# ctpeterson/qex

Hardware: AMD Instinct MI355X
Metric: staggered Dslash GFLOP/s + CG iters/s, 32^4 SU(3) fp64, 1/2/4/8 MI355X (higher is better)
Workload: dtype f64

## Files before the change

profiles/summarize.py:

```python
import csv
import glob
import json
import os
import re
import shutil
import sys
from collections import defaultdict

outdir, tag = sys.argv[1], sys.argv[2]
VOL = 32 ** 4
for d in sorted(glob.glob(os.path.join(outdir, "trace_*"))):
    name = os.path.basename(d)[len("trace_"):]
    for f in glob.glob(os.path.join(d, "**", "*kernel_stats.csv"), recursive=True):
        shutil.copy(f, os.path.join(outdir, "%s_%s_kernel_stats.csv" % (tag, name)))


def split_name(full):
    s = full.strip()
    s = re.sub(r"^void\s+", "", s)
    m = re.match(r"([A-Za-z_][A-Za-z0-9_:]*)", s)
    fn = m.group(1) if m else s
    rest = s[len(fn):]
    targs = ""
    if rest.startswith("<"):
# ... 65 lines not shown
    return (tot / n, n, lo, hi) if n else (None, 0, None, None)


GiB = 1024.0 ** 3
rd, _ = mean("k_read16", None, "FETCH_SIZE")
cp_w, _ = mean("k_copy16", None, "WRITE_SIZE")
if rd and cp_w:
    fcorr = GiB / (rd * 1024.0)
    wcorr = GiB / (cp_w * 1024.0)
    note = ("HBM bytes per launch = FETCH_SIZE*1024*fetch_correction + WRITE_SIZE*1024*write_correction, dispatch-weighted means over "
            "the dispatches of profiles/pmc_workload.py; corrections from the 1 GiB k_read16 / k_copy16 kernels of the same passes; "
            "kernels matched by exact function name and template arguments")
    tj = {"source": "profiles/collect.sh " + tag, "fetch_correction": fcorr, "write_correction": wcorr, "note": note}
    for fn, targs, key in (("k_dslash", "<8, false, false, false, 0>", "dslash8_sweep1_18real"), ("k_dslash", "<8, false, true, true, 0>", "dslash8_sweep2_18real"),
                           ("k_dslash", "<8, false, false, false, 1>", "dslash8_sweep1_recon12"), ("k_dslash", "<8, false, true, true, 1>", "dslash8_sweep2_recon12"),
                           ("k_dslash", "<16, false, false, false, 0>", "dslash16_sweep1_18real"), ("k_dslash", "<16, false, true, true, 0>", "dslash16_sweep2_18real")):
        fe, _ = mean(fn, targs, "FETCH_SIZE")
        wr, _ = mean(fn, targs, "WRITE_SIZE")
        if fe is not None and wr is not None:
            tj[key + "_bytes"] = fe * 1024.0 * fcorr + wr * 1024.0 * wcorr
    if "dslash8_sweep1_18real_bytes" in tj and "dslash8_sweep2_18real_bytes" in tj:
        tj["hbm_bytes_per_launch_32x4"] = 0.5 * (tj["dslash8_sweep1_18real_bytes"] + tj["dslash8_sweep2_18real_bytes"])
    if "dslash8_sweep1_recon12_bytes" in tj and "dslash8_sweep2_recon12_bytes" in tj:
        tj["hbm_bytes_per_launch_32x4_recon12"] = 0.5 * (tj["dslash8_sweep1_recon12_bytes"] + tj["dslash8_sweep2_recon12_bytes"])
    json.dump(tj, open(os.path.join(outdir, "%s_dslash_traffic.json" % tag), "w"), indent=1)

    Vh = VOL // 2
    M = 144
    priced = [
        ("k_dslash", "<8, false, false, false, 0>", (8 * M + 48 + 48) * Vh, "8 links + vector in + vector out per output site (SURVEY 8d: 1248 B)"),
        ("k_dslash", "<8, false, true, true, 0>", (8 * M + 48 + 48 + 48) * Vh, "the same + the 4 m^2 x term (1296 B)"),
        ("k_dslash", "<16, false, false, false, 0>", (16 * M + 48 + 48) * Vh, "16 links + vector in + out (2400 B)"),
        ("k_dslash", "<16, false, true, true, 0>", (16 * M + 48 + 48 + 48) * Vh, "the same + the 4 m^2 x term"),
        ("k_cg_xpay", None, 144 * Vh, "p = r + beta p: 2 reads + 1 write of 48 B"),
        ("k_cg_update", None, 288 * Vh, "x, r updates: 4 reads + 2 writes of 48 B"),
        ("k_cgm_update", None, (48 + 96 + 9 * 192) * Vh, "r in, ps[0] in/out, 9 x (xs, ps in/out), 10 shifts"),
        ("k_force_lds", None, (4 * M * 3 + 4 * M * 2.0 / 3.0) * VOL, "U in, U' out, momentum out, momentum in for stages 2-3 (2112 B/site average)"),
        ("k_force_lds2", None, (4 * M * 3 + 4 * M * 2.0 / 3.0) * VOL, "U in, U' out, momentum out, momentum in for stages 2-3 (2112 B/site average); both parities of a tile position per workgroup"),
        ("k_plaq", None, 4 * M * VOL, "4 links per site read once (576 B)"),
        ("k_flow_obs_clover", None, 4 * M * VOL, "4 links per site read once (576 B)"),
        ("k_flow_obs_clover2", None, 4 * M * VOL, "4 links per site read once (576 B): plaquettes + clover E, Q in one pass, both parities of a tile position per workgroup"),
        ("k_flow_obs_all", None, 4 * M * VOL, "4 links per site read once (576 B): plaquette + clover E, Q in one pass"),
        ("k_gen_staple", None, 4 * M * VOL, "two input matrices read once, accumulator read + written: 576 B/site unique"),
        ("k_staple_deriv_pair", None, 10 * M * VOL, "a (mu,nu)/(nu,mu) pair: 6 matrices read, 2 read and written back = 1440 B/site (rounds 2-3 quoted the 8 reads alone, 1152 B, against read + write traffic)"),
        ("k_projUderiv_batch", None, None, "864 B per link of the batch (sizes differ per level: see dispatches)"),
    ]
    kt = {"source": "profiles/collect.sh " + tag + " (profiles/pmc_workload.py, 32^4)", "fetch_correction": fcorr, "write_correction": wcorr,
          "note": note + "; avg_us from the --kernel-trace --stats pass of the same workload; achieved_alg_gbs = alg_bytes / avg_us", "kernels": {}}
    for fn, targs, alg, what in priced:
        fe, nfe = mean(fn, targs, "FETCH_SIZE")
        wr, _ = mean(fn, targs, "WRITE_SIZE")
        if fe is None or wr is None:
            continue
        hbm_r, hbm_w = fe * 1024.0 * fcorr, wr * 1024.0 * wcorr
        us, ncalls, lo, hi = avg_us(fn, targs)
        e = {"dispatches_pmc": nfe, "hbm_read_bytes": round(hbm_r), "hbm_write_bytes": round(hbm_w), "hbm_bytes": round(hbm_r + hbm_w), "what_alg_counts": what}
        if alg is not None:
            e["alg_bytes"] = int(alg)
            e["ratio_hbm_over_alg"] = round((hbm_r + hbm_w) / alg, 3)
        if us:
            e.update({"avg_us": round(us, 2), "min_us": round(lo, 2), "max_us": round(hi, 2), "calls_trace": ncalls})
            if alg is not None:
                e["achieved_alg_gbs"] = round(alg / us / 1e3, 1)
                e["frac_of_8TBs"] = round(alg / us / 1e3 / 8000.0, 4)
            e["achieved_hbm_gbs"] = round((hbm_r + hbm_w) / us / 1e3, 1)
        for extra in ("TCC_HIT_sum", "TCC_MISS_sum", "TCP_TCC_READ_REQ_sum"):
            v, _ = mean(fn, targs, extra)
            if v is not None:
# ... 5 lines not shown
```

qex_amd/csrc/api.cpp:

```cpp
#include "qexhip_internal.h"
#include <string>
#include "../../include/qexhip.h"
#include <algorithm>
#include <cmath>
#include <cstdarg>
#include <cstdlib>
#include <cstring>
#include <vector>

static thread_local char g_err[1024] = "";

void qexhip_set_error(const char *fmt, ...) {
  va_list ap;
  va_start(ap, fmt);
  vsnprintf(g_err, sizeof(g_err), fmt, ap);
  va_end(ap);
}
extern "C" const char *qexhip_last_error(void) { return g_err; }

static bool timer_class_on(const qexhip_ctx *c, const char *name) {
  if (!c->timers_on) return false;
  if (c->timers_on == 2) return strncmp(name, "dslash", 6) == 0;
  if (c->timers_on == 3) return strncmp(name, "dslash", 6) == 0 || strcmp(name, "exchange") == 0 || strcmp(name, "allreduce") == 0;
  return true;
// ... 57 lines not shown
  return 0;
}

static int init_body(qexhip_ctx *c, int device, const int latLocal[4], const int rankGeom[4], const int rankCoord[4]) {
  int ndev = 0;
  HIPCHK(hipGetDeviceCount(&ndev));
  if (ndev <= 0) { qexhip_set_error("no HIP device visible: libqexhip has no CPU fallback"); return QEXHIP_ERR_HIP; }
  if (device < 0 || device >= ndev) { qexhip_set_error("device %d out of range (%d visible)", device, ndev); return QEXHIP_ERR_ARG; }
  c->device = device;
  for (int i = 0; i < 4; i++) {
    c->rankGeom[i] = rankGeom ? rankGeom[i] : 1;
    c->rankCoord[i] = rankCoord ? rankCoord[i] : 0;
  }
  for (int i = 0; i < 3; i++)
    if (c->rankGeom[i] != 1) { qexhip_set_error("only rankGeom = {1,1,1,N} (split along t) is supported"); return QEXHIP_ERR_ARG; }
  const int halo = c->rankGeom[3] > 1;
  if (geom_init(c->g, latLocal, 1, halo)) return QEXHIP_ERR_ARG;
  HIPCHK(hipSetDevice(device));
  HIPCHK(hipStreamCreateWithFlags(&c->stream, hipStreamNonBlocking));
  {
    int lo = 0, hi = 0;
    if (hipDeviceGetStreamPriorityRange(&lo, &hi) == hipSuccess && hi != lo) HIPCHK(hipStreamCreateWithPriority(&c->cstream, hipStreamNonBlocking, hi));
    else HIPCHK(hipStreamCreateWithFlags(&c->cstream, hipStreamNonBlocking));
  }
  HIPCHK(hipEventCreateWithFlags(&c->ev_ready, hipEventDisableTiming));
  c->part2_off = std::max(6144, (c->g.Vh + 255) / 256 + 8);
  c->npartials = c->part2_off + 2048 + 64;
  HIPCHK(hipMalloc((void **)&c->partials, sizeof(double) * c->npartials));
  HIPCHK(hipMalloc((void **)&c->dscal, sizeof(double) * 64));
  HIPCHK(hipMemset(c->dscal, 0, sizeof(double) * 64));
  HIPCHK(hipMalloc((void **)&c->cg, sizeof(CgScal)));
  HIPCHK(hipMemset(c->cg, 0, sizeof(CgScal)));
  HIPCHK(hipHostMalloc(&c->pinned, 4096, hipHostMallocDefault));
  CHK(devjoin_init(c));
  if (getenv("QEXHIP_TEST_FAIL_INIT")) {
    qexhip_set_error("QEXHIP_TEST_FAIL_INIT: injected failure");
    return QEXHIP_ERR_HIP;
  }
  if (const char *e = getenv("QEXHIP_OVERLAP")) c->opt_overlap = atoi(e);
  if (const char *e = getenv("QEXHIP_HOP_SPLIT")) { const int v = atoi(e); c->opt_hop_split = v < 0 ? -1 : (v ? 2 : 0); }
  if (const char *e = getenv("QEXHIP_RECON")) c->opt_recon = atoi(e);
  if (const char *e = getenv("QEXHIP_FLOW_EXP")) c->opt_flow_exp = atoi(e);
  {
    int a = 0, b = 0;
    (void)hipDeviceGetAttribute(&a, hipDeviceAttributeMaxSharedMemoryPerBlock, device);
    (void)hipDeviceGetAttribute(&b, hipDeviceAttributeSharedMemPerBlockOptin, device);
    (void)hipGetLastError();
    const int lds = a > b ? a : b;
    if (lds < 147456 + 1024) {
      qexhip_set_error("device %d offers %d bytes of LDS per workgroup; libqexhip is built for gfx950 (160 KiB)", device, lds);
      return QEXHIP_ERR_STATE;
    }
  }
  c->nranks = 1;
  c->rank = 0;
  return 0;
}

extern "C" int qexhip_init(qexhip_handle *h, int device, const int latLocal[4], const int rankGeom[4],
                           const int rankCoord[4]) {
  if (!h || !latLocal) return QEXHIP_ERR_ARG;
  qexhip_ctx *c = new qexhip_ctx();
  const int e = init_body(c, device, latLocal, rankGeom, rankCoord);
  if (e) {
    (void)qexhip_finalize(c);
    return e;
// ... 19 lines not shown
  for (auto &kv : c->timers) for (auto e : kv.second.ev) (void)hipEventDestroy(e);
  nhyp_state_free(c);
  hisq_state_free(c);
  batch_state_free(c);
  batch_f32_state_free(c);
  batch_half_state_free(c);
  msf_state_free(c);
  gfix_state_free(c);
  stout_state_free(c);
  eig_state_free(c);
  eig_bases_free(c);
  for (auto &kv : c->cfields) (void)hipFree(kv.second.d);
  c->cfields.clear();
  gauge_free(c);
  comm_destroy(c);
  if (c->W) (void)hipFree(c->W);
  f32_state_free(c);
  half_state_free(c);
  if (c->outer_F) (void)hipFree(c->outer_F);
  if (c->obs_table) (void)hipFree(c->obs_table);
  if (c->tile_order) (void)hipFree(c->tile_order);
  for (int *&t : c->tile_order_pl) if (t) { (void)hipFree(t); t = nullptr; }
  if (c->cgm_scal) (void)hipFree(c->cgm_scal);
  if (c->meson_buf) (void)hipFree(c->meson_buf);
  if (c->Wc) (void)hipFree(c->Wc);
  if (c->Ws) (void)hipFree(c->Ws);
  if (c->Wm) (void)hipFree(c->Wm);
  if (c->stage) (void)hipFree(c->stage);
  if (c->partials) (void)hipFree(c->partials);
  if (c->dscal) (void)hipFree(c->dscal);
  if (c->cg) (void)hipFree(c->cg);
  if (c->hist) (void)hipFree(c->hist);
  if (c->pinned) (void)hipHostFree(c->pinned);
  if (c->fz_buf) (void)hipFree(c->fz_buf);
  devjoin_destroy(c);
  if (c->ev_ready) (void)hipEventDestroy(c->ev_ready);
  if (c->stream) (void)hipStreamDestroy(c->stream);
  if (c->cstream) (void)hipStreamDestroy(c->cstream);
  (void)hipGetLastError();
  delete c;
  return 0;
}

extern "C" int qexhip_sync(qexhip_handle c) {
  if (!c) return QEXHIP_ERR_ARG;
  CHK(devjoin_flush(c));
  HIPCHK(hipStreamSynchronize(c->cstream));
  HIPCHK(hipStreamSynchronize(c->stream));
  return devjoin_check(c);
}

extern "C" int qexhip_device_info(qexhip_handle c, char *buf, int buflen) {
  if (!c || !buf) return QEXHIP_ERR_ARG;
  hipDeviceProp_t p;
  HIPCHK(hipGetDeviceProperties(&p, c->device));
  int n = snprintf(buf, buflen, "%s (%s) CUs=%d mem=%.0fGiB local=%dx%dx%dx%d ranks=%d halo=%d tile_pairs=%d", p.name, p.gcnArchName,
                   p.multiProcessorCount, p.totalGlobalMem / 1073741824.0, c->g.X[0], c->g.X[1], c->g.X[2], c->g.X[3],
                   c->rankGeom[3], c->g.halo, c->tile_order ? c->tile_pairs_ok : -1);
  if (c->g.halo && c->W && n > 0 && n < buflen) {
    double t[8];
    if (qexhip_stag_sweep_tuning(c, t) == 0)
      snprintf(buf + n, buflen - n, "; sweep: overlap=%d form=%s exchange=%.1fus%s boundary_at=%.2f spin=%.0fus tuned[first|sites|fused]=%.0f|%.0f|%.0f us",
               (int)t[7], t[5] == 2 ? "fused" : "by-sites", t[0], c->xchg_us[c->ndir == 16] > 0 ? "(measured)" : "(estimate)", t[1], t[6], t[2], t[3], t[4]);
  }
  return 0;
}
// ... 1438 lines not shown
```

qex_amd/csrc/blas.hip:

```cpp
#include "qexhip_internal.h"
#include "reduce.h"
#include "cg_device.h"
#include <cstring>
#include "peer_device.h"

static inline int grid_for(size_t n2) {
  size_t nb = (n2 + 255) / 256;
  if (nb > 2048) nb = 2048;
  if (nb < 1) nb = 1;
  return (int)nb;
}
static inline size_t body2(const qexhip_ctx *c) { return (size_t)c->g.ntile * 192; }

#define FOR_PAR(par, p) for (int p = ((par) == 2 ? 0 : (par)); p <= ((par) == 2 ? 1 : (par)); p++)

__global__ void __launch_bounds__(256) k_zero(double2 *y, size_t n) {
  for (size_t i = blockIdx.x * 256 + threadIdx.x; i < n; i += (size_t)gridDim.x * 256) y[i] = make_double2(0, 0);
}
__global__ void __launch_bounds__(256) k_copy(double2 *y, const double2 *x, size_t n) {
  for (size_t i = blockIdx.x * 256 + threadIdx.x; i < n; i += (size_t)gridDim.x * 256) y[i] = x[i];
}
__global__ void __launch_bounds__(256) k_axpy(double a, const double2 *x, double2 *y, size_t n) {
  for (size_t i = blockIdx.x * 256 + threadIdx.x; i < n; i += (size_t)gridDim.x * 256) {
    double2 xv = x[i], yv = y[i];
// ... 137 lines not shown
  if (threadIdx.x == 0) out[blockIdx.x] = r;
}
int blas_cdot(qexhip_ctx *c, const DevField &x, const DevField &y, int parity, double *dev_out) {
  size_t n = body2(c);
  const int nb = grid_for(n);
  int tot = 0;
  double *pre = c->partials, *pim = c->partials + 2 * nb;
  if (4 * nb > c->part2_off + 2048) { qexhip_set_error("internal: partial buffer too small for cdot"); return -3; }
  {
    ScopedTimer tm(c, "blas", c->stream);
    FOR_PAR(parity, p) {
      k_cdot<<<nb, 256, 0, c->stream>>>(x.par(p), y.par(p), n, pre + tot, pim + tot);
      tot += nb;
    }
    k_reduce_final2<<<2, 256, 0, c->stream>>>(pre, pim, tot, dev_out);
    HIPCHK(hipGetLastError());
  }
  if (multi_rank(c)) CHK(comm_allreduce(c, dev_out, 2));
  return 0;
}

int blas_norm2(qexhip_ctx *c, const DevField &x, int parity, double *dev_out) {
  return blas_redot(c, x, x, parity, dev_out);
}

int read_scalars(qexhip_ctx *c, const double *dev, int n, double *host) {
  HIPCHK(hipMemcpyAsync(c->pinned, dev, sizeof(double) * n, hipMemcpyDeviceToHost, c->stream));
  HIPCHK(hipStreamSynchronize(c->stream));
  CHK(peer_check(c));
  for (int i = 0; i < n; i++) host[i] = ((double *)c->pinned)[i];
  return 0;
}

__global__ void __launch_bounds__(256) k_cg_xpay(double2 *p, const double2 *r, size_t n, CgScal *s, int k, int rolled,
                                                const double *r2parts, int nparts, double *hist, int histcap) {
  const int cur = k & 1, prv = cur ^ 1;
  double r2k;
  if (rolled) {
    if (s->dones[cur]) return;
    r2k = s->r2s[cur];
  } else {
    if (s->dones[prv]) {
      if (blockIdx.x == 0 && threadIdx.x == 0) cg_carry(s, k);
      return;
    }
    r2k = cg_sum_parts(r2parts, nparts);
    if (blockIdx.x == 0 && threadIdx.x == 0) cg_roll(s, k, r2k, hist, histcap);
    if (!(k < s->maxits && r2k > s->r2stop)) return;
  }
  const bool first = (k == 0);
  const double beta = r2k / s->r2s[prv];
  for (size_t i = blockIdx.x * 256 + threadIdx.x; i < n; i += (size_t)gridDim.x * 256) {
    double2 rv = r[i];
    if (first) p[i] = rv;
    else {
      double2 pv = p[i];
      p[i] = make_double2(fma(beta, pv.x, rv.x), fma(beta, pv.y, rv.y));
    }
  }
}
__global__ void __launch_bounds__(256) k_cg_update(double2 *x, double2 *r, const double2 *p, const double2 *Ap,
                                                  size_t n, const CgScal *s, int k, double *partials,
                                                  const double *dotp, int ndot) {
  if (s->dones[k & 1]) return;
  const double pAp = (ndot > 0) ? cg_sum_parts(dotp, ndot) : s->pAp;
  const double alpha = s->r2s[k & 1] / pAp;
  double acc = 0;
  for (size_t i = blockIdx.x * 256 + threadIdx.x; i < n; i += (size_t)gridDim.x * 256) {
    double2 pv = p[i], xv = x[i], rv = r[i], av = Ap[i];
    xv.x += alpha * pv.x; xv.y += alpha * pv.y;
    rv.x -= alpha * av.x; rv.y -= alpha * av.y;
    x[i] = xv; r[i] = rv;
    acc = fma(rv.x, rv.x, fma(rv.y, rv.y, acc));
  }
  double t = block_sum_256(acc);
  if (threadIdx.x == 0) partials[blockIdx.x] = t;
}
__global__ void k_cg_init(CgScal *s, const double *dscal, double r2req, int maxits, double *hist, int histcap) {
  s->b2 = dscal[0];
  s->r2 = dscal[1];
  s->rzo = 1.0;
  s->pAp = 0.0;
  s->r2stop = r2req * s->b2;
  s->itn = 0;
  s->maxits = maxits;
  s->done = !(0 < maxits && s->r2 > s->r2stop);
  s->r2s[0] = s->r2; s->itns[0] = 0; s->dones[0] = s->done;
  s->r2s[1] = 1.0; s->itns[1] = 0; s->dones[1] = s->done;
  if (histcap > 0) hist[0] = (s->b2 != 0.0) ? s->r2 / s->b2 : 0.0;
}
__global__ void __launch_bounds__(256) k_cg_close(CgScal *s, int k, const double *r2parts, int nparts, double *hist, int histcap) {
  if (s->dones[(k & 1) ^ 1]) {
    if (threadIdx.x == 0) cg_carry(s, k);
    return;
  }
  const double r2k = cg_sum_parts(r2parts, nparts);
  if (threadIdx.x == 0) cg_roll(s, k, r2k, hist, histcap);
}

int cg_xpay(qexhip_ctx *c, DevField &p, const DevField &r, int parity, int k, int rolled) {
  size_t n = body2(c);
  ScopedTimer tm(c, "blas", c->stream);
  k_cg_xpay<<<grid_for(n), 256, 0, c->stream>>>(p.par(parity), r.par(parity), n, c->cg, k, rolled,
                                               c->partials + c->part2_off, rolled ? grid_for(n) : c->cg_r2parts, c->hist, c->histcap);
  HIPCHK(hipGetLastError());
  return 0;
}
int cg_update(qexhip_ctx *c, DevField &x, DevField &r, const DevField &p, const DevField &Ap, int parity, int k, int ndot) {
  size_t n = body2(c);
  int nb = grid_for(n);
  double *r2p = c->partials + c->part2_off;
  if (ndot > 0) CHK(comm_allreduce_parts(c, c->partials, ndot, &ndot));
  CHK(devjoin_flush(c));
  {
    ScopedTimer tm(c, "blas", c->stream);
    k_cg_update<<<nb, 256, 0, c->stream>>>(x.par(parity), r.par(parity), p.par(parity), Ap.par(parity), n, c->cg, k, r2p,
                                           c->partials, ndot);
    HIPCHK(hipGetLastError());
  }
  CHK(comm_allreduce_parts(c, r2p, nb, &c->cg_r2parts));
  return 0;
}
int cg_close(qexhip_ctx *c, int k) {
  k_cg_close<<<1, 256, 0, c->stream>>>(c->cg, k, c->partials + c->part2_off, c->cg_r2parts, c->hist, c->histcap);
  HIPCHK(hipGetLastError());
  return comm_agree_post(c);
}
__global__ void k_cg_resume(CgScal *s, int k, double r2req, int maxits) {
  const int cur = k & 1;
  s->r2stop = r2req * s->b2;
  s->maxits = maxits;
  s->r2s[cur] = s->r2; s->r2s[cur ^ 1] = s->rzo; s->itns[cur] = k;
  s->dones[cur] = !(k < maxits && s->r2s[cur] > s->r2stop);
  s->done = s->dones[cur];
  s->agree[0] = s->r2s[cur]; s->agree[1] = -s->r2s[cur]; s->agree[2] = (double)k; s->agree[3] = -(double)k;
}
int cg_resume(qexhip_ctx *c, int k, double r2req, int maxits) {
  k_cg_resume<<<1, 1, 0, c->stream>>>(c->cg, k, r2req, maxits);
  HIPCHK(hipGetLastError());
  return 0;
}
int cg_init(qexhip_ctx *c, double r2req, int maxits) {
  c->cg_resume.valid = 0;
  k_cg_init<<<1, 1, 0, c->stream>>>(c->cg, c->dscal, r2req, maxits, c->hist, c->histcap);
  HIPCHK(hipGetLastError());
  return 0;
}
```

qex_amd/csrc/qexhip_internal.h:

```cpp
#pragma once
#include <hip/hip_runtime.h>
#include <cstdint>
#include <cstdio>
#include <string>
#include <vector>
#include <map>

#define QEXHIP_TILE 64

struct Geom {
  int X[4];
  int Xh;
  int V, Vh;
  int F;
  int ntile;
  int depth;
  int gtile;
  int etile;
  int halo;
};

__host__ __device__ inline size_t vec_off(int pos, int colour) {
  return (size_t)(pos >> 6) * 192 + (size_t)colour * 64 + (size_t)(pos & 63);
}
// ... 7 lines not shown
  double2 *d = nullptr;
  size_t half = 0;
  double2 *par(int p) const { return d + (size_t)p * half; }
};

struct DevFieldF {
  float2 *d = nullptr;
  size_t half = 0;
  float2 *par(int p) const { return d + (size_t)p * half; }
};

struct DevCField {
  double2 *d = nullptr;
  size_t half = 0;
  double2 *par(int p) const { return d + (size_t)p * half; }
};

struct SlpScal {
  double b2, r2stop;
  double r2t;
  double sigma, sigma_p;
  double r2s, r2s_old, maxr2s;
  int k, maxits, nupd;
  int done, upd, noupd;
  int conv, first;
};

struct CgScal {
  double b2, r2, rzo, pAp, r2stop, tmp;
  int itn, maxits, done, pad;
  double r2s[2];
  int itns[2], dones[2];
  double agree[4];
};

struct TimerSlot {
  std::vector<hipEvent_t> ev;
  size_t used = 0;
  long count = 0;
  double total_ms = 0;
};

struct DevJoin {
  unsigned long long *ready = nullptr;
  unsigned long long *err = nullptr;
  long long ticks = 0;
  double timeout_s = 30.0;
  unsigned long long seq[2]{0, 0};
  int deferred = 0;
};

struct GaugeNat {
  double2 *U = nullptr, *F = nullptr, *P = nullptr;
  double2 *U2 = nullptr;
  double2 *D2 = nullptr;
  size_t n2 = 0;
  int ghost_valid = 0;
  double *pp = nullptr; int npp = 0;
  double2 *M = nullptr;
  double2 *Usave = nullptr;
  int save_ghost_valid = 0;
};
struct PeerComm;

struct EigBasis {
  double2 *v = nullptr;
// ... 2 lines not shown
  unsigned long gen = 0;
  std::vector<double> evals;
  int nevals = 0;
};

enum { WK_SLOTS = 16 };

struct qexhip_ctx {
  int device = 0;
  Geom g{};
  int rankGeom[4]{1, 1, 1, 1}, rankCoord[4]{0, 0, 0, 0};
  hipStream_t stream = nullptr, cstream = nullptr;
  hipEvent_t ev_ready = nullptr;
  void *comm = nullptr;
  void *comm2 = nullptr;
  PeerComm *peer = nullptr;
  DevJoin dj;
  int opt_transport = -1;
  int nranks = 1, rank = 0;
  int force_halo = 0;
  double2 *W = nullptr;
  int ndir = 0;
  std::map<int, DevField> fields;
  int next_field = 1;
  double *stage = nullptr; size_t stage_bytes = 0;
  double *partials = nullptr; int npartials = 0;
  int part2_off = 0;
  double *dscal = nullptr;
  CgScal *cg = nullptr;
  struct { int valid = 0; const double2 *x = nullptr; int par_even = 0; double m2 = 0; int k = 0; } cg_resume;
  int cg_r2parts = 0;
  double *hist = nullptr; int histcap = 0;
  void *pinned = nullptr;
  int wk[WK_SLOTS]{0};
  int timers_on = 0;
  std::map<std::string, TimerSlot> timers;
  double2 *Wc = nullptr; unsigned long long *Ws = nullptr; size_t Wc_rows = 0; int recon = 0; double recon_dev = 0;
  unsigned long long *Wm = nullptr; size_t Wm_rows = 0; int lres = 0; long long lres_esc = 0;
  int opt_lossless = 3;
  int opt_batch_multi = 0;
  int opt_multi_reduce = 0;
  int opt_force_pair = 1;
  int opt_obs_clover = 1;
  int opt_hop_split = -1;
  int opt_fused_spin_us = -1;
  int ranks_share_device = 0;
  int hybrid_sums = 0;
  unsigned int *fz_buf = nullptr; int fz_cap = 0;
  const double2 *bnd_out_on_cstream = nullptr;
  double xchg_us[2]{0, 0};
  int form_auto[2]{-1, -1};
  int opt_chain_overlap = 1;
  int opt_hisq_md_fused = 3;
  int opt_smear_ca = 1;
  int opt_flow_exp = 1;
  int opt_recon = 2;
  int opt_overlap = -1;
  int emu_link_gbs = 0;
  int emu_exchange_us = 0, emu_allreduce_us = 0;
  int overlap_auto[2]{-1, -1};
  double overlap_tune_us[2][3]{};
  GaugeNat *gn = nullptr;
  void *nhyp = nullptr;
  void *hisq = nullptr;
  double2 *outer_F = nullptr; size_t outer_Fn = 0;
  int tile_pairs_ok = 0;
// ... 181 lines not shown
int half_pack_host(const double *v, size_t nsites, int16_t *q, float *norm);
int half_unpack_host(const int16_t *q, const float *norm, size_t nsites, double *v);
int half_links(qexhip_ctx *c, int *fmt, double *s_fat, double *s_long, double *dev);
int half_op_xx_probe(qexhip_ctx *c, DevField &fr, const DevField &fx, double m2, int par_even);
int slph_begin(qexhip_ctx *c, SlpScal *s);
int slph_iterate(qexhip_ctx *c, SlpScal *s, DevFieldF &xs, const DevField &r, double m2, int par_even);
int slph_stall(qexhip_ctx *c, SlpScal *s, int limit);
int slph_stalled(qexhip_ctx *c, int *stalled);
void half_state_free(qexhip_ctx *c);

#define CGM_MAXM 32
void msf_state_free(qexhip_ctx *c);
int msf_r2_buffer(qexhip_ctx *c, double **dev);
int msf_start(qexhip_ctx *c, SlpScal *s, DevFieldF &rs, const DevField &b, std::vector<DevField *> &xs, const double *shifts, int nmass,
              int parity, DevFieldF **ps0);
int msf_iterate(qexhip_ctx *c, SlpScal *s, DevFieldF &rs, const DevFieldF &Ap, const DevField &r, int parity, int ndot);
int msf_flush(qexhip_ctx *c, SlpScal *s, int nmass);

int blas_zero(qexhip_ctx *c, DevField &f, int parity);
int blas_copy(qexhip_ctx *c, DevField &dst, const DevField &src, int parity);
int blas_axpy(qexhip_ctx *c, double a, const DevField &x, DevField &y, int parity);
int blas_xpay(qexhip_ctx *c, const DevField &x, double a, DevField &y, int parity);
int blas_scale(qexhip_ctx *c, double a, DevField &y, int parity);
int blas_axpby(qexhip_ctx *c, double a, const DevField &x, double b, const DevField &y, DevField &z, int parity);
int blas_norm2(qexhip_ctx *c, const DevField &x, int parity, double *dev_out);
int blas_redot(qexhip_ctx *c, const DevField &x, const DevField &y, int parity, double *dev_out);
int blas_cdot(qexhip_ctx *c, const DevField &x, const DevField &y, int parity, double *dev_out);
int tile_order_table(qexhip_ctx *c, const int **tab, int *chunk);
int tile_order_plane(qexhip_ctx *c, int mu, int nu, const int **tab, int *chunk);
int reduce_partials(qexhip_ctx *c, int n, double *dev_out);
int read_scalars(qexhip_ctx *c, const double *dev, int n, double *host);
int blas_grid(const qexhip_ctx *c, int parity_count);
int blas_delay(hipStream_t st, int us);
int cg_xpay(qexhip_ctx *c, DevField &p, const DevField &r, int parity, int k, int rolled);
int cg_update(qexhip_ctx *c, DevField &x, DevField &r, const DevField &p, const DevField &Ap, int parity, int k, int ndot);
int cg_close(qexhip_ctx *c, int k);
int cg_init(qexhip_ctx *c, double r2req, int maxits);
int cg_resume(qexhip_ctx *c, int k, double r2req, int maxits);

int get_work(qexhip_ctx *c, int slot, DevField **f);
int op_xx(qexhip_ctx *c, DevField &r, DevField &x, double m2, int par_even, int dot, const int *done, int *ndot = nullptr);
int op_D(qexhip_ctx *c, DevField &r, DevField &x, double m, double sc, double a = 0.0);
int norm2_eo(qexhip_ctx *c, DevField &f, double *e, double *o);
int resid_eo(qexhip_ctx *c, DevField &r, DevField &b, DevField &x, double m, double *e, double *o);
int solve_xx_dev(qexhip_ctx *c, DevField &x, DevField &b, double mass, double r2req, int maxits,
                 int par_even, int *iters, double *r2_over_b2, double *hist, int histcap);
int solve_xx_continue_dev(qexhip_ctx *c, DevField &x, double r2req, int maxits, int *iters, double *r2_over_b2, double *hist, int histcap);
int solve_full_dev(qexhip_ctx *c, DevField &x, DevField &b, double mass, double r2req, int maxits,
                   int *iters, double *r2_final, int use_prev = 0, int sloppy = 0, int *nupdates = nullptr);
int solve_xx_sloppy_dev(qexhip_ctx *c, DevField &x, DevField &b, double mass, double r2req, int maxits, int par_even,
                        int *iters, double *r2_over_b2, int *nupdates);
int solve_xx_half_dev(qexhip_ctx *c, DevField &x, DevField &b, double mass, double r2req, int maxits, int par_even,
                      int *iters, double *r2_over_b2, int *nupdates);
int half_finish_f32(qexhip_ctx *c, DevField &x, DevField &b, const DevField &r, DevField &Ax, double mass, double r2stop, int maxits,
                    int par_even, double *r2t, int *its32, int *nupd32);
int solve_xx_sloppy_any(qexhip_ctx *c, int sloppy, DevField &x, DevField &b, double mass, double r2req, int maxits, int par_even,
                        int *iters, double *r2_over_b2, int *nupdates);
int solve_xx_multi_dev(qexhip_ctx *c, std::vector<DevField *> &xs, DevField &b, const double *shifts,
                       int nmass, double r2req, int maxits, int par_even, int *iters, double *hist, int histcap);
int solve_multi_dev(qexhip_ctx *c, std::vector<DevField *> &xs, DevField &b, const double *masses,
                    int nmass, double r2req, int maxits, int *iters, double *r2_final, int sloppy = 0, int *nupdates = nullptr);
int multi_sloppy_check(qexhip_ctx *c, int sloppy, const double *vals, int nmass);
int solve_xx_multi_sloppy_dev(qexhip_ctx *c, std::vector<DevField *> &xs, DevField &b, const double *shifts, int nmass, double r2req,
                              int maxits, int par_even, int *iters, double *r2_over_b2, int *nupdates, int *refine_iters);
enum { POOL_PS = 0, POOL_YS = 32, POOL_XS = 64, POOL_REF = 96 };
int pool_field(qexhip_ctx *c, int idx, DevField **f);
int rational_map(const char *who, double mass, int nterm, const double *alpha, const double *beta, double *shifts, int *order);
int rational_xx_dev(qexhip_ctx *c, DevField &out, DevField &b, double mass, double f0, int nterm, const double *alpha, const double *beta,
                    double r2req, int maxits, int par_even, int *iters, double *hist, int histcap);
// ... 127 lines not shown
```

qex_amd/csrc/solver.cpp:

```cpp
#include "qexhip_internal.h"
#include "full_solve.h"
#include "../../include/qexhip.h"
#include <cmath>
#include <cstring>
#include <algorithm>
#include <vector>


int get_work(qexhip_ctx *c, int slot, DevField **f) {
  if (slot == WK_R || slot == WK_P || slot == WK_AP) c->cg_resume.valid = 0;
  if (c->wk[slot] == 0) {
    DevField nf;
    CHK(field_alloc(c, nf));
    int id = -(slot + 1);
    c->fields[id] = nf;
    c->wk[slot] = id;
  }
  *f = &c->fields[c->wk[slot]];
  return 0;
}

int op_xx(qexhip_ctx *c, DevField &r, DevField &x, double m2, int par_even, int dot, const int *done, int *ndot) {
  DevField *t;
  CHK(get_work(c, WK_T, &t));
  const int px = par_even ? 0 : 1, py = 1 - px;
  DslashOpts o1, o2;
  o1.done = done;
  o2.cb = 4.0 * m2;
  o2.xs = &x;
  o2.neg = 1;
  o2.dot = (dot && ndot) ? 2 : dot;
  o2.nparts_out = ndot;
  o2.dot_out = &c->cg->pAp;
  o2.done = done;
// ... 16 lines not shown
}

int op_D(qexhip_ctx *c, DevField &r, DevField &x, double m, double sc, double a) {
  CHK(op_stagD(c, r, x, 0, m, sc, a));
  CHK(op_stagD(c, r, x, 1, m, sc, a));
  return 0;
}

static int op_eo_reconstruct(qexhip_ctx *c, DevField &r, DevField &b, double m) {
  CHK(op_stagD(c, r, r, 1, 0.0, -1.0 / m, 0.0));
  CHK(blas_axpy(c, 1.0 / m, b, r, 1));
  return 0;
}
int op_eo_reconstruct_pub(qexhip_ctx *c, DevField &r, DevField &b, double m) { return op_eo_reconstruct(c, r, b, m); }
int op_stagD_pub(qexhip_ctx *c, DevField &r, DevField &x, int parity, double m, double sc, double a) { return op_stagD(c, r, x, parity, m, sc, a); }
int op_eo_reduce_pub(qexhip_ctx *c, DevField &r, DevField &b, double m) { return op_stagD(c, r, b, 0, m, -1.0, 0.0); }

static int ensure_hist(qexhip_ctx *c, int cap) {
  if (cap < 1) cap = 1;
  if (c->histcap >= cap) return 0;
  if (c->hist) HIPCHK(hipFree(c->hist));
  c->hist = nullptr; c->histcap = 0;
  HIPCHK(hipMalloc((void **)&c->hist, sizeof(double) * cap));
  c->histcap = cap;
  return 0;
}

static int read_cg(qexhip_ctx *c, CgScal *host) {
  HIPCHK(hipMemcpyAsync(c->pinned, c->cg, sizeof(CgScal), hipMemcpyDeviceToHost, c->stream));
  HIPCHK(hipStreamSynchronize(c->stream));
  memcpy(host, c->pinned, sizeof(CgScal));
  return 0;
}

static int cg_iterate(qexhip_ctx *c, DevField &x, DevField *r, DevField *p, DevField *Ap, double m2, int par_even, int k,
                      CgScal &st, int *iters, double *r2_over_b2, double *hist, int histcap) {
  const int par = par_even ? 0 : 1;
  const int chunk = 32;
  int rolled = 1;
  bool done = st.dones[k & 1];
  double r2 = st.r2s[k & 1];
  st.itn = st.itns[k & 1];
  while (!done) {
    int n = std::min(chunk, st.maxits - k);
    if (n <= 0) break;
    for (int i = 0; i < n; i++, k++) {
      CHK(cg_xpay(c, *p, *r, par, k, rolled));
      rolled = 0;
      int ndot = 0;
      CHK(op_xx(c, *Ap, *p, m2, par_even, 1, &c->cg->dones[k & 1], &ndot));
      CHK(cg_update(c, x, *r, *p, *Ap, par, k, ndot));
    }
    CHK(cg_close(c, k));
    rolled = 1;
    CHK(read_cg(c, &st));
    CHK(comm_agree_check(c, st));
    done = st.dones[k & 1];
    r2 = st.r2s[k & 1];
    st.itn = st.itns[k & 1];
  }
  st.r2 = r2;
  if (iters) *iters = st.itn;
  if (r2_over_b2) *r2_over_b2 = (st.b2 != 0.0) ? st.r2 / st.b2 : 0.0;
  if (hist && histcap > 0) {
    int n = std::min(std::min(histcap, c->histcap), st.itn + 1);
    HIPCHK(hipMemcpyAsync(hist, c->hist, sizeof(double) * n, hipMemcpyDeviceToHost, c->stream));
    HIPCHK(hipStreamSynchronize(c->stream));
  }
  c->cg_resume.valid = 1; c->cg_resume.x = x.d; c->cg_resume.par_even = par_even; c->cg_resume.m2 = m2; c->cg_resume.k = st.itn;
  return 0;
}

int solve_xx_dev(qexhip_ctx *c, DevField &x, DevField &b, double mass, double r2req, int maxits,
                 int par_even, int *iters, double *r2_over_b2, double *hist, int histcap) {
  const int par = par_even ? 0 : 1;
  DevField *r, *p, *Ap;
  CHK(get_work(c, WK_R, &r));
  CHK(get_work(c, WK_P, &p));
  CHK(get_work(c, WK_AP, &Ap));
  CHK(ensure_hist(c, std::max(histcap, 1)));
  const double m2 = mass * mass;
  CHK(blas_zero(c, x, 2));
  CHK(blas_norm2(c, b, par, &c->dscal[0]));
  CHK(blas_copy(c, *r, b, par));
  CHK(blas_norm2(c, *r, par, &c->dscal[1]));
  CHK(cg_init(c, r2req, maxits));
  CgScal st;
  CHK(read_cg(c, &st));
  return cg_iterate(c, x, r, p, Ap, m2, par_even, 0, st, iters, r2_over_b2, hist, histcap);
}

int solve_xx_continue_dev(qexhip_ctx *c, DevField &x, double r2req, int maxits, int *iters, double *r2_over_b2, double *hist, int histcap) {
// ... 527 lines not shown
```

Before: 3012.

## Defer CG x update into next xpay and post chunk-end reads ahead

The CG x += alpha p update moves out of k_cg_update into the next iteration's k_cg_xpay, or into k_cg_close at a chunk end. alpha is stored in CgScal for that purpose. This shrinks the update kernel's traffic and fuses the x stream with the p stream. The chunk-end host read of the CG scalars now goes through an event with double-buffered pinned slots, and two iterations of the next chunk are enqueued before the host waits, so the GPU does not sit idle during the convergence check. The cost is a close kernel that now sweeps the whole field, and up to two extra speculative iterations, which are gated on device by the done flags.

```diff
diff --git a/profiles/summarize.py b/profiles/summarize.py
--- a/profiles/summarize.py
+++ b/profiles/summarize.py
@@ -121,8 +121,8 @@
         ("k_dslash", "<8, false, true, true, 0>", (8 * M + 48 + 48 + 48) * Vh, "the same + the 4 m^2 x term (1296 B)"),
         ("k_dslash", "<16, false, false, false, 0>", (16 * M + 48 + 48) * Vh, "16 links + vector in + out (2400 B)"),
         ("k_dslash", "<16, false, true, true, 0>", (16 * M + 48 + 48 + 48) * Vh, "the same + the 4 m^2 x term"),
-        ("k_cg_xpay", None, 144 * Vh, "p = r + beta p: 2 reads + 1 write of 48 B"),
-        ("k_cg_update", None, 288 * Vh, "x, r updates: 4 reads + 2 writes of 48 B"),
+        ("k_cg_xpay", None, 240 * Vh, "x += alpha p of the iteration before, p = r + beta p: 3 reads + 2 writes of 48 B"),
+        ("k_cg_update", None, 144 * Vh, "r update: 2 reads + 1 write of 48 B"),
         ("k_cgm_update", None, (48 + 96 + 9 * 192) * Vh, "r in, ps[0] in/out, 9 x (xs, ps in/out), 10 shifts"),
         ("k_force_lds", None, (4 * M * 3 + 4 * M * 2.0 / 3.0) * VOL, "U in, U' out, momentum out, momentum in for stages 2-3 (2112 B/site average)"),
         ("k_force_lds2", None, (4 * M * 3 + 4 * M * 2.0 / 3.0) * VOL, "U in, U' out, momentum out, momentum in for stages 2-3 (2112 B/site average); both parities of a tile position per workgroup"),
diff --git a/qex_amd/csrc/api.cpp b/qex_amd/csrc/api.cpp
--- a/qex_amd/csrc/api.cpp
+++ b/qex_amd/csrc/api.cpp
@@ -113,6 +113,7 @@
   HIPCHK(hipMalloc((void **)&c->cg, sizeof(CgScal)));
   HIPCHK(hipMemset(c->cg, 0, sizeof(CgScal)));
   HIPCHK(hipHostMalloc(&c->pinned, 4096, hipHostMallocDefault));
+  for (hipEvent_t &e : c->cg_ev) HIPCHK(hipEventCreateWithFlags(&e, hipEventDisableTiming));
   CHK(devjoin_init(c));
   if (getenv("QEXHIP_TEST_FAIL_INIT")) {
     qexhip_set_error("QEXHIP_TEST_FAIL_INIT: injected failure");
@@ -198,6 +199,7 @@
   if (c->cg) (void)hipFree(c->cg);
   if (c->hist) (void)hipFree(c->hist);
   if (c->pinned) (void)hipHostFree(c->pinned);
+  for (hipEvent_t e : c->cg_ev) if (e) (void)hipEventDestroy(e);
   if (c->fz_buf) (void)hipFree(c->fz_buf);
   devjoin_destroy(c);
   if (c->ev_ready) (void)hipEventDestroy(c->ev_ready);
diff --git a/qex_amd/csrc/blas.hip b/qex_amd/csrc/blas.hip
--- a/qex_amd/csrc/blas.hip
+++ b/qex_amd/csrc/blas.hip
@@ -193,46 +193,80 @@
   return 0;
 }
 
-__global__ void __launch_bounds__(256) k_cg_xpay(double2 *p, const double2 *r, size_t n, CgScal *s, int k, int rolled,
+
+__device__ __forceinline__ double2 cg_xup(double alpha, double2 pv, double2 xv) {
+  return make_double2(fma(alpha, pv.x, xv.x), fma(alpha, pv.y, xv.y));
+}
+
+__global__ void __launch_bounds__(256) k_cg_xpay(double2 *x, double2 *p, const double2 *r, size_t n, CgScal *s, int k, int rolled,
                                                 const double *r2parts, int nparts, double *hist, int histcap) {
   const int cur = k & 1, prv = cur ^ 1;
-  double r2k;
+  const size_t stride = (size_t)gridDim.x * 256;
+  size_t i = blockIdx.x * 256 + threadIdx.x;
+  const bool first = (k == 0), pend = !rolled;
+  double2 rv = make_double2(0, 0), pv = rv, xv = rv;
+  if (i < n) {
+    rv = r[i];
+    if (!first) pv = p[i];
+    if (pend) xv = x[i];
+  }
+  const int done_prv = s->dones[prv], maxits = s->maxits;
+  const double r2prv = s->r2s[prv], r2stop = s->r2stop, alpha = s->alphas[prv];
+  const int done_cur = rolled ? s->dones[cur] : 0;
+  double r2k = rolled ? s->r2s[cur] : 0.0;
+  bool go = true;
   if (rolled) {
-    if (s->dones[cur]) return;
-    r2k = s->r2s[cur];
+    if (done_cur) return;
   } else {
-    if (s->dones[prv]) {
+    if (done_prv) {
       if (blockIdx.x == 0 && threadIdx.x == 0) cg_carry(s, k);
       return;
     }
     r2k = cg_sum_parts(r2parts, nparts);
     if (blockIdx.x == 0 && threadIdx.x == 0) cg_roll(s, k, r2k, hist, histcap);
-    if (!(k < s->maxits && r2k > s->r2stop)) return;
-  }
-  const bool first = (k == 0);
-  const double beta = r2k / s->r2s[prv];
-  for (size_t i = blockIdx.x * 256 + threadIdx.x; i < n; i += (size_t)gridDim.x * 256) {
-    double2 rv = r[i];
+    go = (k < maxits && r2k > r2stop);
+  }
+  if (!go) {
+    while (i < n) {
+      x[i] = cg_xup(alpha, pv, xv);
+      i += stride;
+      if (i < n) { pv = p[i]; xv = x[i]; }
+    }
+    return;
+  }
+  const double beta = r2k / r2prv;
+  while (i < n) {
+    if (pend) x[i] = cg_xup(alpha, pv, xv);
     if (first) p[i] = rv;
-    else {
-      double2 pv = p[i];
-      p[i] = make_double2(fma(beta, pv.x, rv.x), fma(beta, pv.y, rv.y));
-    }
-  }
-}
-__global__ void __launch_bounds__(256) k_cg_update(double2 *x, double2 *r, const double2 *p, const double2 *Ap,
-                                                  size_t n, const CgScal *s, int k, double *partials,
+    else p[i] = make_double2(fma(beta, pv.x, rv.x), fma(beta, pv.y, rv.y));
+    i += stride;
+    if (i < n) {
+      rv = r[i];
+      if (!first) pv = p[i];
+      if (pend) xv = x[i];
+    }
+  }
+}
+__global__ void __launch_bounds__(256) k_cg_update(double2 *r, const double2 *Ap, size_t n, CgScal *s, int k, double *partials,
                                                   const double *dotp, int ndot) {
-  if (s->dones[k & 1]) return;
-  const double pAp = (ndot > 0) ? cg_sum_parts(dotp, ndot) : s->pAp;
-  const double alpha = s->r2s[k & 1] / pAp;
+  const int cur = k & 1;
+  const size_t stride = (size_t)gridDim.x * 256;
+  size_t i = blockIdx.x * 256 + threadIdx.x;
+  double2 rv = make_double2(0, 0), av = rv;
+  if (i < n) { rv = r[i]; av = Ap[i]; }
+  const int done = s->dones[cur];
+  const double r2 = s->r2s[cur], pAp0 = s->pAp;
+  if (done) return;
+  const double pAp = (ndot > 0) ? cg_sum_parts(dotp, ndot) : pAp0;
+  const double alpha = r2 / pAp;
+  if (blockIdx.x == 0 && threadIdx.x == 0) s->alphas[cur] = alpha;
   double acc = 0;
-  for (size_t i = blockIdx.x * 256 + threadIdx.x; i < n; i += (size_t)gridDim.x * 256) {
-    double2 pv = p[i], xv = x[i], rv = r[i], av = Ap[i];
-    xv.x += alpha * pv.x; xv.y += alpha * pv.y;
+  while (i < n) {
     rv.x -= alpha * av.x; rv.y -= alpha * av.y;
-    x[i] = xv; r[i] = rv;
+    r[i] = rv;
     acc = fma(rv.x, rv.x, fma(rv.y, rv.y, acc));
+    i += stride;
+    if (i < n) { rv = r[i]; av = Ap[i]; }
   }
   double t = block_sum_256(acc);
   if (threadIdx.x == 0) partials[blockIdx.x] = t;
@@ -250,24 +284,39 @@
   s->r2s[1] = 1.0; s->itns[1] = 0; s->dones[1] = s->done;
   if (histcap > 0) hist[0] = (s->b2 != 0.0) ? s->r2 / s->b2 : 0.0;
 }
-__global__ void __launch_bounds__(256) k_cg_close(CgScal *s, int k, const double *r2parts, int nparts, double *hist, int histcap) {
-  if (s->dones[(k & 1) ^ 1]) {
-    if (threadIdx.x == 0) cg_carry(s, k);
+__global__ void __launch_bounds__(256) k_cg_close(double2 *x, const double2 *p, size_t n, CgScal *s, int k, const double *r2parts,
+                                                 int nparts, double *hist, int histcap) {
+  const int prv = (k & 1) ^ 1;
+  const size_t stride = (size_t)gridDim.x * 256;
+  size_t i = blockIdx.x * 256 + threadIdx.x;
+  double2 pv = make_double2(0, 0), xv = pv;
+  if (i < n) { pv = p[i]; xv = x[i]; }
+  const int done_prv = s->dones[prv];
+  const double alpha = s->alphas[prv];
+  if (done_prv) {
+    if (blockIdx.x == 0 && threadIdx.x == 0) cg_carry(s, k);
     return;
   }
-  const double r2k = cg_sum_parts(r2parts, nparts);
-  if (threadIdx.x == 0) cg_roll(s, k, r2k, hist, histcap);
-}
-
-int cg_xpay(qexhip_ctx *c, DevField &p, const DevField &r, int parity, int k, int rolled) {
+  if (blockIdx.x == 0) {
+    const double r2k = cg_sum_parts(r2parts, nparts);
+    if (threadIdx.x == 0) cg_roll(s, k, r2k, hist, histcap);
+  }
+  while (i < n) {
+    x[i] = cg_xup(alpha, pv, xv);
+    i += stride;
+    if (i < n) { pv = p[i]; xv = x[i]; }
+  }
+}
+
+int cg_xpay(qexhip_ctx *c, DevField &x, DevField &p, const DevField &r, int parity, int k, int rolled) {
   size_t n = body2(c);
   ScopedTimer tm(c, "blas", c->stream);
-  k_cg_xpay<<<grid_for(n), 256, 0, c->stream>>>(p.par(parity), r.par(parity), n, c->cg, k, rolled,
+  k_cg_xpay<<<grid_for(n), 256, 0, c->stream>>>(x.par(parity), p.par(parity), r.par(parity), n, c->cg, k, rolled,
                                                c->partials + c->part2_off, rolled ? grid_for(n) : c->cg_r2parts, c->hist, c->histcap);
   HIPCHK(hipGetLastError());
   return 0;
 }
-int cg_update(qexhip_ctx *c, DevField &x, DevField &r, const DevField &p, const DevField &Ap, int parity, int k, int ndot) {
+int cg_update(qexhip_ctx *c, DevField &r, const DevField &Ap, int parity, int k, int ndot) {
   size_t n = body2(c);
   int nb = grid_for(n);
   double *r2p = c->partials + c->part2_off;
@@ -275,15 +324,16 @@
   CHK(devjoin_flush(c));
   {
     ScopedTimer tm(c, "blas", c->stream);
-    k_cg_update<<<nb, 256, 0, c->stream>>>(x.par(parity), r.par(parity), p.par(parity), Ap.par(parity), n, c->cg, k, r2p,
-                                           c->partials, ndot);
+    k_cg_update<<<nb, 256, 0, c->stream>>>(r.par(parity), Ap.par(parity), n, c->cg, k, r2p, c->partials, ndot);
     HIPCHK(hipGetLastError());
   }
   CHK(comm_allreduce_parts(c, r2p, nb, &c->cg_r2parts));
   return 0;
 }
-int cg_close(qexhip_ctx *c, int k) {
-  k_cg_close<<<1, 256, 0, c->stream>>>(c->cg, k, c->partials + c->part2_off, c->cg_r2parts, c->hist, c->histcap);
+int cg_close(qexhip_ctx *c, DevField &x, const DevField &p, int parity, int k) {
+  size_t n = body2(c);
+  k_cg_close<<<grid_for(n), 256, 0, c->stream>>>(x.par(parity), p.par(parity), n, c->cg, k, c->partials + c->part2_off, c->cg_r2parts,
+                                                c->hist, c->histcap);
   HIPCHK(hipGetLastError());
   return comm_agree_post(c);
 }
diff --git a/qex_amd/csrc/cg_posting.h b/qex_amd/csrc/cg_posting.h
--- /dev/null
+++ b/qex_amd/csrc/cg_posting.h
@@ -0,0 +1,28 @@
+#pragma once
+#include <vector>
+
+enum { CG_POST_ITERS = 0, CG_POST_CLOSE = 1, CG_POST_WAIT = 2 };
+struct CgPostStep {
+  int kind, k, n;
+};
+
+inline std::vector<CgPostStep> cg_posting_plan(int k, int maxits, int chunk, int ahead) {
+  std::vector<CgPostStep> plan;
+  if (chunk < 1) chunk = 1;
+  if (ahead < 0) ahead = 0;
+  if (ahead > chunk) ahead = chunk;
+  int n = maxits - k < chunk ? maxits - k : chunk;
+  if (n <= 0) return plan;
+  plan.push_back({CG_POST_ITERS, k, n});
+  k += n;
+  for (;;) {
+    plan.push_back({CG_POST_CLOSE, k, 0});
+    n = maxits - k < chunk ? maxits - k : chunk;
+    const int a = n < ahead ? (n > 0 ? n : 0) : ahead;
+    if (a > 0) plan.push_back({CG_POST_ITERS, k, a});
+    plan.push_back({CG_POST_WAIT, k, 0});
+    if (n <= 0) return plan;
+    if (n > a) plan.push_back({CG_POST_ITERS, k + a, n - a});
+    k += n;
+  }
+}
diff --git a/qex_amd/csrc/qexhip_internal.h b/qex_amd/csrc/qexhip_internal.h
--- a/qex_amd/csrc/qexhip_internal.h
+++ b/qex_amd/csrc/qexhip_internal.h
@@ -63,6 +63,7 @@
   double r2s[2];
   int itns[2], dones[2];
   double agree[4];
+  double alphas[2];
 };
 
 struct TimerSlot {
@@ -131,6 +132,7 @@
   int cg_r2parts = 0;
   double *hist = nullptr; int histcap = 0;
   void *pinned = nullptr;
+  hipEvent_t cg_ev[2]{nullptr, nullptr};
   int wk[WK_SLOTS]{0};
   int timers_on = 0;
   std::map<std::string, TimerSlot> timers;
@@ -378,9 +380,9 @@
 int read_scalars(qexhip_ctx *c, const double *dev, int n, double *host);
 int blas_grid(const qexhip_ctx *c, int parity_count);
 int blas_delay(hipStream_t st, int us);
-int cg_xpay(qexhip_ctx *c, DevField &p, const DevField &r, int parity, int k, int rolled);
-int cg_update(qexhip_ctx *c, DevField &x, DevField &r, const DevField &p, const DevField &Ap, int parity, int k, int ndot);
-int cg_close(qexhip_ctx *c, int k);
+int cg_xpay(qexhip_ctx *c, DevField &x, DevField &p, const DevField &r, int parity, int k, int rolled);
+int cg_update(qexhip_ctx *c, DevField &r, const DevField &Ap, int parity, int k, int ndot);
+int cg_close(qexhip_ctx *c, DevField &x, const DevField &p, int parity, int k);
 int cg_init(qexhip_ctx *c, double r2req, int maxits);
 int cg_resume(qexhip_ctx *c, int k, double r2req, int maxits);
 
diff --git a/qex_amd/csrc/solver.cpp b/qex_amd/csrc/solver.cpp
--- a/qex_amd/csrc/solver.cpp
+++ b/qex_amd/csrc/solver.cpp
@@ -1,5 +1,6 @@
 #include "qexhip_internal.h"
 #include "full_solve.h"
+#include "cg_posting.h"
 #include "../../include/qexhip.h"
 #include <cmath>
 #include <cstring>
@@ -82,32 +83,52 @@
   memcpy(host, c->pinned, sizeof(CgScal));
   return 0;
 }
+static_assert(sizeof(CgScal) <= 512, "two CgScal slots in the pinned scratch");
+static int post_read_cg(qexhip_ctx *c, int slot) {
+  HIPCHK(hipMemcpyAsync((char *)c->pinned + 512 * slot, c->cg, sizeof(CgScal), hipMemcpyDeviceToHost, c->stream));
+  HIPCHK(hipEventRecord(c->cg_ev[slot], c->stream));
+  return 0;
+}
+static int wait_read_cg(qexhip_ctx *c, int slot, CgScal *host) {
+  HIPCHK(hipEventSynchronize(c->cg_ev[slot]));
+  memcpy(host, (char *)c->pinned + 512 * slot, sizeof(CgScal));
+  return 0;
+}
 
 static int cg_iterate(qexhip_ctx *c, DevField &x, DevField *r, DevField *p, DevField *Ap, double m2, int par_even, int k,
                       CgScal &st, int *iters, double *r2_over_b2, double *hist, int histcap) {
   const int par = par_even ? 0 : 1;
   const int chunk = 32;
+  const int ahead = 2;
   int rolled = 1;
   bool done = st.dones[k & 1];
   double r2 = st.r2s[k & 1];
   st.itn = st.itns[k & 1];
-  while (!done) {
-    int n = std::min(chunk, st.maxits - k);
-    if (n <= 0) break;
-    for (int i = 0; i < n; i++, k++) {
-      CHK(cg_xpay(c, *p, *r, par, k, rolled));
-      rolled = 0;
-      int ndot = 0;
-      CHK(op_xx(c, *Ap, *p, m2, par_even, 1, &c->cg->dones[k & 1], &ndot));
-      CHK(cg_update(c, x, *r, *p, *Ap, par, k, ndot));
-    }
-    CHK(cg_close(c, k));
-    rolled = 1;
-    CHK(read_cg(c, &st));
-    CHK(comm_agree_check(c, st));
-    done = st.dones[k & 1];
-    r2 = st.r2s[k & 1];
-    st.itn = st.itns[k & 1];
+  if (!done) {
+    int slot = 0;
+    for (const CgPostStep &ps : cg_posting_plan(k, st.maxits, chunk, ahead)) {
+      if (ps.kind == CG_POST_ITERS) {
+        for (k = ps.k; k < ps.k + ps.n; k++) {
+          CHK(cg_xpay(c, x, *p, *r, par, k, rolled));
+          rolled = 0;
+          int ndot = 0;
+          CHK(op_xx(c, *Ap, *p, m2, par_even, 1, &c->cg->dones[k & 1], &ndot));
+          CHK(cg_update(c, *r, *Ap, par, k, ndot));
+        }
+      } else if (ps.kind == CG_POST_CLOSE) {
+        CHK(cg_close(c, x, *p, par, ps.k));
+        rolled = 1;
+        slot ^= 1;
+        CHK(post_read_cg(c, slot));
+      } else {
+        CHK(wait_read_cg(c, slot, &st));
+        CHK(comm_agree_check(c, st));
+        done = st.dones[ps.k & 1];
+        r2 = st.r2s[ps.k & 1];
+        st.itn = st.itns[ps.k & 1];
+        if (done) break;
+      }
+    }
   }
   st.r2 = r2;
   if (iters) *iters = st.itn;
diff --git a/scratch/timeline_chunk_end.py b/scratch/timeline_chunk_end.py
--- /dev/null
+++ b/scratch/timeline_chunk_end.py
@@ -0,0 +1,44 @@
+import csv, glob, statistics, sys
+d = sys.argv[1]
+f = glob.glob(d + "/**/*kernel_trace.csv", recursive=True)[0]
+rows = list(csv.DictReader(open(f)))
+short = lambda n: n.split("(")[0].replace("void ", "")[:44]
+ev = sorted((int(r["Start_Timestamp"]), int(r["End_Timestamp"]), short(r["Kernel_Name"])) for r in rows)
+cg = ("k_cg_xpay", "k_dslash", "k_cg_update", "k_cg_close")
+closes = [i for i, e in enumerate(ev) if e[2].startswith("k_cg_close")]
+spans = []
+for i in closes:
+    nxt = [j for j in range(i + 1, min(i + 8, len(ev))) if ev[j][2].startswith("k_cg_xpay")]
+    if not ev[i - 1][2].startswith("k_cg_update") or not nxt:
+        continue
+    j = nxt[0]
+    if any(not (ev[m][2].startswith("__amd_rocclr_copyBuffer")) for m in range(i + 1, j)):
+        continue
+    busy = sum(ev[m][1] - ev[m][0] for m in range(i, j))
+    spans.append((i, j, (ev[j][0] - ev[i - 1][1] - busy) / 1e3, (ev[j][0] - ev[i - 1][1]) / 1e3))
+print("chunk ends inside a solve: %d" % len(spans))
+if spans:
+    idle = [s[2] for s in spans]
+    wall = [s[3] for s in spans]
+    print("  update end -> next xpay start: median %.1f us (min %.1f, max %.1f); of it idle (no kernel running): median %.1f us (min %.1f, max %.1f)"
+          % (statistics.median(wall), min(wall), max(wall), statistics.median(idle), min(idle), max(idle)))
+    which = int(sys.argv[2]) if len(sys.argv) > 2 else len(spans) - 1
+    i, j = spans[which][0], spans[which][1]
+    t0 = ev[i - 4][0]
+    print("  one of them (start, end, duration, gap in front; us):")
+    for m in range(i - 4, min(j + 5, len(ev))):
+        s, e, n = ev[m]
+        print("  %9.1f %9.1f  %7.1f  gap %6.1f  %s" % ((s - t0) / 1e3, (e - t0) / 1e3, (e - s) / 1e3, (s - ev[m - 1][1]) / 1e3, n))
+gaps, durs = {}, {}
+for a, b in zip(ev, ev[1:]):
+    if a[2].startswith(cg) and b[2].startswith(cg) and not a[2].startswith("k_cg_close") and not b[2].startswith("k_cg_close"):
+        gaps.setdefault(a[2][:28] + " -> " + b[2][:28], []).append((b[0] - a[1]) / 1e3)
+for e in ev:
+    if e[2].startswith(cg) and e[1] - e[0] > 4000:
+        durs.setdefault(e[2], []).append((e[1] - e[0]) / 1e3)
+print("median gap per boundary inside an iteration (us):")
+for k, v in gaps.items():
+    print("  %-62s %6.2f  (n %d)" % (k, statistics.median(v), len(v)))
+print("median duration of the live launches (us):")
+for k, v in durs.items():
+    print("  %-44s %6.2f  (n %d)" % (k, statistics.median(v), len(v)))
```

After: 3130 (median of 6 runs). +3.9%, better.
